# smn-ailab/PyCMF

Hardware: AMD Instinct MI355X
Metric: factor-update iterations/s (mu solver: one full update_step per iteration) (higher is better)
Workload: dtype f32

## Files before the change

pycmf_amd/csrc/cmf_api.hip:

```cpp
#include "../../include/cmfhip.h"
#include "cmf_kernels.hip.h"
#include "cmf_gemm_pair.hip.h"
#include "cmf_eigen.hip.h"
#include "cmf_chol_mfma.hip.h"
#include "cmf_sparse.hip.h"
#include "cmf_rowhess.hip.h"
#include "cmf_bf16x6.hip.h"
#include "cmf_rowhess6.hip.h"
#include "cmf_shared64.hip.h"
#include "cmf_refine64.hip.h"
#include "cmf_eigclamp.hip.h"
#include "cmf_rank1clamp.hip.h"

#include <hip/hip_runtime.h>

#include <algorithm>
#include <chrono>
#include <cmath>
#include <cstdarg>
#include <cstdio>
#include <cstdlib>
#include <cstring>
#include <mutex>
#include <numeric>
#include <set>
#include <string>
#include <thread>
#include <vector>

using namespace cmfk;

static thread_local std::string g_err;

static int fail(int code, const char *fmt, ...) {
    char buf[512];
    va_list ap;
    va_start(ap, fmt);
    vsnprintf(buf, sizeof buf, fmt, ap);
    va_end(ap);
    g_err = buf;
    return code;
}

#define HIPCHK(expr)                                                                       \
    do {                                                                                   \
        hipError_t e_ = (expr);                                                            \
        if (e_ != hipSuccess)                                                              \
            return fail(e_ == hipErrorOutOfMemory ? CMF_ENOMEM : CMF_EHIP, "%s failed: %s (%s:%d)", \
                        #expr, hipGetErrorString(e_), __FILE__, __LINE__);                 \
    } while (0)
#define CHK(expr)                 \
    do {                          \
        int rc_ = (expr);         \
        if (rc_ != CMF_OK) return rc_; \
    } while (0)

static inline int64_t rup(int64_t x, int64_t a) { return (x + a - 1) / a * a; }

struct DevBuf {
    void *p = nullptr;
    size_t bytes = 0;
};

struct CsrDev {
    int64_t *indptr = nullptr;
    int32_t *idx = nullptr;
    float *val = nullptr;
    int64_t rows = 0, cols = 0, nnz = 0;
    cmfk::BcsrEntry *b_ent = nullptr;
    int64_t *b_seg = nullptr;
    int32_t *b_grow = nullptr;
    int b_ngroups = 0, b_nblocks = 0, b_rows_per_group = 0, b_nsync = 1;
    int32_t *b_vmap = nullptr, *b_prow = nullptr, *b_pfirst = nullptr, *b_pcnt = nullptr;
    int b_nsplit = 0, b_nslots = 0;
};

struct WCsrDev {
    int64_t *indptr = nullptr;
    int32_t *idx = nullptr;
    float *pv = nullptr, *wv = nullptr, *tv = nullptr;
    float *ev = nullptr;
    int64_t rows = 0, cols = 0, nnz = 0;
};

struct StepGraph {
    hipGraphExec_t exec = nullptr;
    double key[8] = {0};
    int warm = 0;
    bool failed = false;
};

struct EvPair {
    hipEvent_t a, b;
    int cls;
    double flops;
};

struct CmfComm;
struct cmf_ctx {
    int device = 0;
    CmfComm *comm = nullptr;
    hipStream_t stream = nullptr;
    bool own_stream = false;
    int num_cu = 256;

    int64_t m = 0, d = 0, p = 0;
    int k = 0;
    int64_t mp = 0, dp = 0, pp = 0;
    int kp = 0;
    bool have_problem = false;
    unsigned long long *dbg_stamps = nullptr;
    bool diag_ok = false;
    int opt_graph = -1;
    StepGraph mu_graph, newton_graph;
    int opt_split = -1;
    int opt_pair = 1;
    int opt_arith_min_tiles = 8;
    int opt_arith = 0;
    int opt_ns = 1;
    bool hess_psd = true;
    int opt_pipe_nt = 4;
    int opt_topk_split = 0;
    int opt_kl_split = 0;
    DevBuf kl_slab, kl_small, kl_part;
    int opt_wmu_split = 0;
    int wm_kind[2] = {0, 0};
    float *wm_w[2] = {nullptr, nullptr}, *wm_p[2] = {nullptr, nullptr};
    WCsrDev wm_sp[2][2];
    DevBuf wm_slab, wm_small, wm_part;
    DevBuf hals_ws;
    int opt_als_piece = 0;
    DevBuf als_h, als_part, als_g, als_sol, als_desc;
    DevBuf als_nnls_ws;
    int opt_als_cg_lds = -1;
    DevBuf als_cg_ws;
    int opt_als_cg_piece = 0;
    DevBuf als_cg_long;
    int64_t als_cg_last[2] = {0, 0};
    double wm_bg[2] = {0.0, 0.0};
    DevBuf als_bg_s, als_bg64;
    int opt_choldiag = 0;
    int opt_chol = 1;
    int opt_chol_mfma = 1;
    int opt_zlogit_l2 = 1;
    int opt_rowdiag = 0;
    int opt_rowsym = 4;
    int opt_rowstagger = 1;
    int opt_rowkernel = 1;
    double flop_scale = 1.0;
    bool dev_sampling = false;
    uint64_t dev_seed = 0;
    int64_t sample_off[3] = {0, 0, 0};

    float *X = nullptr, *Y = nullptr;
    CsrDev sp[2][2];
    bool sparse[2] = {false, false};
    double sp_sq[2] = {0.0, 0.0};
    int opt_sparse = 0;
    int opt_spmm_blocked = 1;
    int64_t opt_spmm_block_cols = 0;
    int64_t opt_spmm_stretch = 0;
    DevBuf spmm_bar;
    DevBuf spmm_part;
    int opt_spmm_split = 1;
    float *F[3] = {nullptr, nullptr, nullptr};
    int64_t frows[3] = {0, 0, 0}, frows_pad[3] = {0, 0, 0};
    int64_t v_rows_alloc = 0;

    float *num = nullptr, *den = nullptr;
    float *G = nullptr, *G2 = nullptr, *Hm = nullptr, *Hinv = nullptr, *Eye = nullptr;
    float *vbuf = nullptr;
    DevBuf gslab32;
    int opt_gram32_shares = 32;
    int opt_gram32 = 1;
    DevBuf slabs, slabs_b;
    int slab_sel = 0;
    int timed_open = 0;
    DevBuf narrow_tmp;
    int opt_narrow_update = 1;
    int opt_fused_mu = 1;
    int opt_small_tile = 1;
    DevBuf resid;
    DevBuf resid2, resid3;
    DevBuf kr1, kr2;
    DevBuf hrows;
    DevBuf mask1, mask2;
    DevBuf lists1, lists2;
    DevBuf hpart;
    int opt_rowsplit = 1;
    DevBuf lr_small, lr_rows;
    int opt_lowrank = 1;
    DevBuf lists1s, lists2s, zerobuf;
    DevBuf cls_idx[2], cls_off[2], cls_cnt[2], cls_pat[2], hclass;
    DevBuf certimg, certflag;
    int opt_direct_step = 1;
    int opt_rowcert = 1;
    int64_t opt_rowchunk = 0;
    int opt_rowclasses = -1;
    DevBuf idxbuf;
    DevBuf eigws;
    DevBuf eigflag, eigcopy;
    DevBuf clampstat;
    DevBuf badbuf, rw64, rh64;
    DevBuf ref_w, ref_w2, ref_g, ref_i, ref_ns;
    int opt_refine_batched = 1;
    std::vector<int> bad_host;
    int opt_refine = 1;
    double opt_refine_ratio = 3.0e3;
    double opt_refine_cond = 1.0e3;
    double opt_refine_tol = 2.0e-5;
    int64_t opt_refine_max = (int64_t)1 << 40;
    int64_t refined_sweep = 0, refined_total = 0;
    DevBuf bfp[2][2], bff;
    bool bfp_valid[2][2] = {{false, false}, {false, false}};
    DevBuf nsidx, nsws;
    DevBuf eigcl_snap;
    DevBuf eigcl_ws, eigcl_log, eigcl_fail;
    int opt_eig_clamp = 1;
    int64_t eig_clamp_rows = 0;
    DevBuf r1_ws;
    int opt_rank1_clamp = 1;
    int64_t rank1_rows = 0;
    DevBuf g64a, g64b, gmix64, h64;
    DevBuf gslab64, w64, ns64;
    bool gmix64_valid = false;
    int opt_shared64 = 1;
    DevBuf hinv64, opr;
    int opt_reassoc = 1;
    bool v_plain = false;
    DevBuf dpart;
    int opt_trace_error_off = 0;
    bool mu_dots = false;
    DevBuf trace64;
    double dsq_cache[2] = {0.0, 0.0};
    bool dsq_valid[2] = {false, false};
    double *dscalar = nullptr;
    double rh_credited = 0.0, rh_gathered = 0.0;
    std::vector<void *> owned;
    std::vector<void *> scratch;
    std::set<const void *> lds_opt_in;

    int timing = 0;
    std::vector<EvPair> pending;
    std::vector<hipEvent_t> evpool;
    double ms[CMF_K_END] = {0};
    int64_t launches[CMF_K_END] = {0};
    double flops[CMF_K_END] = {0};
    std::vector<hipEvent_t> markers;
    void *pin[2] = {nullptr, nullptr};
    hipEvent_t pin_ev[2] = {nullptr, nullptr};
    bool pin_busy[2] = {false, false};
    double sp_sum[2] = {0.0, 0.0};
};

struct DeviceGuard {
    int prev = -1;
    explicit DeviceGuard(int dev) {
        (void)hipGetDevice(&prev);
        if (prev != dev) (void)hipSetDevice(dev);
        else prev = -1;
    }
    ~DeviceGuard() {
        if (prev >= 0) (void)hipSetDevice(prev);
    }
};

static int ev_get(cmf_ctx *c, hipEvent_t *e) {
    if (!c->evpool.empty()) {
        *e = c->evpool.back();
        c->evpool.pop_back();
        return CMF_OK;
    }
    HIPCHK(hipEventCreate(e));
    return CMF_OK;
}
struct Timed {
    cmf_ctx *c;
    int cls;
    hipEvent_t a = nullptr, b = nullptr;
    bool on = false;
    double flops = 0.0;
    Timed(cmf_ctx *c_, int cls_, double flops_ = 0.0) : c(c_), cls(cls_), flops(flops_) {
        const bool want = c->timed_open == 0 &&
                          (c->timing == 1 || (c->timing == 2 && (cls == CMF_K_GEMM_NN || cls == CMF_K_GEMM_TN || cls == CMF_K_GEMM_PAIR || cls == CMF_K_SPMM || cls == CMF_K_ROWHESS || cls == CMF_K_KLMU)));
        if (want && ev_get(c, &a) == CMF_OK && ev_get(c, &b) == CMF_OK) {
            on = true;
            ++c->timed_open;
            (void)hipEventRecord(a, c->stream);
        }
    }
    ~Timed() {
        if (on) {
            --c->timed_open;
            (void)hipEventRecord(b, c->stream);
            c->pending.push_back({a, b, cls, flops});
        }
    }
};
static int flush_timing(cmf_ctx *c) {
    if (c->pending.empty()) return CMF_OK;
    HIPCHK(hipStreamSynchronize(c->stream));
    for (auto &e : c->pending) {
        float ms = 0.f;
        HIPCHK(hipEventElapsedTime(&ms, e.a, e.b));
        c->ms[e.cls] += ms;
        c->launches[e.cls] += 1;
        c->flops[e.cls] += e.flops;
        c->evpool.push_back(e.a);
        c->evpool.push_back(e.b);
    }
    c->pending.clear();
    return CMF_OK;
}

static int dev_alloc(cmf_ctx *c, void **p, size_t bytes, bool zero = true) {
    HIPCHK(hipMalloc(p, bytes ? bytes : 16));
    c->owned.push_back(*p);
    if (zero) HIPCHK(hipMemsetAsync(*p, 0, bytes ? bytes : 16, c->stream));
    return CMF_OK;
}
static void dev_free(cmf_ctx *c, void *p) {
    if (!p) return;
    auto it = std::find(c->owned.begin(), c->owned.end(), p);
    if (it != c->owned.end()) c->owned.erase(it);
    (void)hipFree(p);
}
static void drop_graph(StepGraph &g) {
    if (g.exec) (void)hipGraphExecDestroy(g.exec);
    g = StepGraph();
}
static void invalidate_graphs(cmf_ctx *c) {
    drop_graph(c->mu_graph);
    drop_graph(c->newton_graph);
}

static int ensure(cmf_ctx *c, DevBuf &b, size_t bytes) {
    if (b.bytes >= bytes) return CMF_OK;
    invalidate_graphs(c);
    if (b.p) {
        HIPCHK(hipStreamSynchronize(c->stream));
        dev_free(c, b.p);
        b.p = nullptr;
        b.bytes = 0;
    }
    CHK(dev_alloc(c, &b.p, bytes, false));
    b.bytes = bytes;
    return CMF_OK;
}

static int allow_big_lds(cmf_ctx *c, const void *fn, int bytes) {
    if (c->lds_opt_in.count(fn)) return CMF_OK;
    HIPCHK(hipFuncSetAttribute(fn, hipFuncAttributeMaxDynamicSharedMemorySize, bytes));
    c->lds_opt_in.insert(fn);
    return CMF_OK;
}

struct GemmPlan {
    int bn;
    int ntiles_n;
    int64_t tiles_m;
    int nsplit;
    int64_t klen;
};

static GemmPlan plan_gemm(const cmf_ctx *c, int64_t mout, int64_t n, int64_t kred, bool allow_split) {
    GemmPlan pl;
    pl.bn = n >= 256 ? 256 : (int)n;
    pl.ntiles_n = (int)(n / pl.bn);
    pl.tiles_m = (mout + 255) / 256;
    const int64_t tiles = pl.tiles_m * pl.ntiles_n;
    int64_t s = 1;
    if (allow_split && c->opt_split > 0) {
        s = std::min<int64_t>(c->opt_split, std::max<int64_t>(1, kred / 32));
    } else if (allow_split && tiles < (int64_t)(c->num_cu * 3) / 4) {
        s = ((int64_t)c->num_cu + tiles / 2) / tiles;
        const int64_t maxs = std::max<int64_t>(1, kred / 128);
        s = std::max<int64_t>(1, std::min(s, maxs));
    }
    pl.klen = rup((kred + s - 1) / s, 32);
    pl.nsplit = (int)((kred + pl.klen - 1) / pl.klen);
    return pl;
}

template <int MODE, int ROLE>
static int launch_gemm(cmf_ctx *c, const GemmArgs &a, const GemmPlan &pl) {
    static_assert(MODE != MODE_NT, "NT passes: gemm_nt");
    dim3 grid((unsigned)pl.tiles_m, (unsigned)pl.ntiles_n, (unsigned)pl.nsplit);
    dim3 block(512);
#define CMF_LAUNCH(BN_)                                                                          \
    do {                                                                                         \
        using Cfg = GemmCfg<MODE, BN_>;                                                          \
        CHK(allow_big_lds(c, reinterpret_cast<const void *>(&gemm_kernel<MODE, BN_, ROLE, 4>), (int)Cfg::LDS_BYTES)); \
        hipLaunchKernelGGL((gemm_kernel<MODE, BN_, ROLE, 4>), grid, block, Cfg::LDS_BYTES, c->stream, a); \
    } while (0)
    switch (pl.bn) {
    case 256: CMF_LAUNCH(256); break;
    case 128: CMF_LAUNCH(128); break;
    case 64: CMF_LAUNCH(64); break;
    case 32: CMF_LAUNCH(32); break;
    default: return fail(CMF_EINVAL, "unsupported tile width %d", pl.bn);
    }
#undef CMF_LAUNCH
    HIPCHK(hipGetLastError());
    return CMF_OK;
}

static int sum_slabs(cmf_ctx *c, float *dst, const float *src, int64_t n, int nslab, int64_t stride,
                     bool accumulate) {
    Timed tm(c, CMF_K_ELEMWISE);
    const int64_t n4 = n / 4;
    const int blocks = (int)std::min<int64_t>((n4 + 255) / 256, 2048);
    hipLaunchKernelGGL(sum_slabs_kernel, dim3(blocks), dim3(256), 0, c->stream, dst, src, n4, nslab, stride,
                       accumulate ? 1 : 0);
    HIPCHK(hipGetLastError());
    return CMF_OK;
}

static int mu_apply(cmf_ctx *c, float *F, const float *num, const float *den, int64_t n, double l1, double l2);

struct SlabRef {
    const float *base = nullptr;
    int nslab = 0;
    int64_t stride = 0;
    int64_t quota = 0, unit0 = 0;
    int ksteps = 0;
};

struct Epilogue {
    int kind = 0;
    const float *F = nullptr, *P = nullptr;
    const SlabRef *Pslabs = nullptr, *Pslabs2 = nullptr;
    float *out = nullptr;
    double a = 0.0, b = 0.0, c = 0.0;
    int64_t rows = 0;
    int kvalid = 0, nn = 0;
};

static int gemm(cmf_ctx *c, int mode, const float *A, int64_t lda, const float *B, int64_t ldb, float *out,
                int64_t mout, int64_t n, int64_t kred, bool accumulate = false, const Epilogue *mu = nullptr, SlabRef *defer = nullptr) {
    const bool data_pass = (lda != c->kp);
    DevBuf &slabbuf = c->slab_sel ? c->slabs_b : c->slabs;
    if (kred % 32 || n % 32) return fail(CMF_EINVAL, "gemm: unpadded extent (k=%lld n=%lld)", (long long)kred, (long long)n);
    GemmPlan pl = plan_gemm(c, mout, n, kred, mu == nullptr);
    if (mu && c->opt_narrow_update && pl.ntiles_n == 1) {
        while (pl.bn > 64 && pl.tiles_m * (n / pl.bn) * 2 <= (int64_t)c->num_cu) pl.bn /= 2;
        pl.ntiles_n = (int)(n / pl.bn);
    }
    float *alias_out = nullptr;
    if (mu && pl.ntiles_n > 1 && mu->out == A) {
        CHK(ensure(c, c->narrow_tmp, (size_t)rup(mout, 256) * n * sizeof(float)));
        alias_out = mu->out;
    }
    GemmArgs a;
    memset(&a, 0, sizeof a);
    a.A = A; a.lda = lda; a.B = B; a.ldb = ldb;
    a.ldc = n;
    a.Mout = (mode == MODE_TN) ? mout : rup(mout, 256);
    a.Kred = kred; a.klen = pl.klen;
    a.dbg = data_pass ? c->dbg_stamps : nullptr;
    const int64_t rows_store = (mode == MODE_TN) ? mout : rup(mout, 256);
    const bool direct = (pl.nsplit == 1 && !accumulate);
    if (mu) {
        if (mode != MODE_NN || pl.nsplit != 1) return fail(CMF_EINVAL, "fused update needs an unsplit NN product");
        a.epi = mu->kind; a.epi_F = mu->F; a.epi_P = mu->P; a.epi_out = alias_out ? (float *)c->narrow_tmp.p : mu->out;
        a.epi_a = (float)mu->a; a.epi_b = (float)mu->b; a.epi_c = (float)mu->c;
        a.epi_rows = mu->rows; a.epi_kvalid = mu->kvalid; a.epi_nn = mu->nn;
        a.C = out;
    } else if (direct) {
        a.C = out;
        a.slab_stride = 0;
    } else if (pl.nsplit == 1) {
        a.red_out = out; a.red_acc = 1;
        a.C = out;
    } else {
        const size_t need = (size_t)pl.nsplit * rows_store * n * sizeof(float);
        CHK(ensure(c, slabbuf, need));
        a.C = (float *)slabbuf.p;
        a.slab_stride = rows_store * n;
    }
    {
        Timed tm(c, !data_pass ? CMF_K_GEMM_SMALL : (mode == MODE_NN ? CMF_K_GEMM_NN : CMF_K_GEMM_TN),
                 2.0 * (double)mout * (double)n * (double)kred * c->flop_scale);
        if (mode == MODE_NN) {
            if (data_pass) CHK((launch_gemm<MODE_NN, 0>(c, a, pl)));
            else CHK((launch_gemm<MODE_NN, 1>(c, a, pl)));
        } else {
            if (data_pass) CHK((launch_gemm<MODE_TN, 0>(c, a, pl)));
            else CHK((launch_gemm<MODE_TN, 1>(c, a, pl)));
        }
    }
    if (alias_out) HIPCHK(hipMemcpyAsync(alias_out, c->narrow_tmp.p, (size_t)rup(mout, 256) * n * sizeof(float), hipMemcpyDeviceToDevice, c->stream));
    if (!mu && pl.nsplit > 1) {
        if (defer && !accumulate) {
            defer->base = (const float *)slabbuf.p; defer->nslab = pl.nsplit; defer->stride = a.slab_stride;
            return CMF_OK;
        }
        CHK(sum_slabs(c, out, (const float *)slabbuf.p, rows_store * n, pl.nsplit, a.slab_stride, accumulate));
    }
    if (defer) *defer = SlabRef();
    return CMF_OK;
}

static int gram32(cmf_ctx *c, const float *F, int64_t rows_pad, float *G) {
    if (!(c->opt_gram32 && (c->kp == 64 || c->kp == 128) && rows_pad >= 1024))
        return gemm(c, MODE_TN, F, c->kp, F, c->kp, G, c->kp, c->kp, rows_pad);
    const int T = c->kp / 64, ntile = T * (T + 1) / 2;
    int64_t nsplit = std::min<int64_t>(std::max<int64_t>(c->opt_gram32_shares, std::min<int64_t>(256, rows_pad / 1024)), rows_pad / 32);
    const int64_t chunk = rup((rows_pad + nsplit - 1) / nsplit, 32);
    nsplit = (rows_pad + chunk - 1) / chunk;
    CHK(ensure(c, c->gslab32, (size_t)nsplit * ntile * 64 * 64 * sizeof(float)));
    Timed tm(c, CMF_K_GEMM_SMALL, 2.0 * (double)rows_pad * c->kp * c->kp);
    hipLaunchKernelGGL(gram32_partial_kernel, dim3((unsigned)ntile, (unsigned)nsplit), dim3(256), 0, c->stream, F, c->kp, rows_pad, chunk, (float *)c->gslab32.p);
    hipLaunchKernelGGL(gram32_reduce_kernel, dim3((unsigned)std::min(64, (c->kp * c->kp + 255) / 256)), dim3(256), 0, c->stream, (const float *)c->gslab32.p,
                       c->kp, (int)nsplit, G);
    HIPCHK(hipGetLastError());
    return CMF_OK;
}

static bool small_tile_ok(const cmf_ctx *c, int64_t rows_pad) {
    return c->opt_fused_mu && c->opt_small_tile && (c->kp == 64 || c->kp == 128) && rows_pad * c->kp <= ((int64_t)1 << 27);
}
static void factor_update_args(FactorUpdArgs &g, const float *A, const float *B, const Epilogue &e) {
    memset(&g, 0, sizeof g);
    g.A = A; g.B = B; g.epi = e.kind; g.F = e.F; g.P = e.P; g.out = e.out;
    if (e.Pslabs && e.Pslabs->nslab > 0) {
        g.S1 = e.Pslabs->base; g.n1 = e.Pslabs->nslab; g.stride1 = e.Pslabs->stride;
        g.q1 = e.Pslabs->quota; g.u1 = e.Pslabs->unit0; g.ks1 = e.Pslabs->ksteps;
    }
    if (e.Pslabs2 && e.Pslabs2->nslab > 0) {
        g.S2 = e.Pslabs2->base; g.n2 = e.Pslabs2->nslab; g.stride2 = e.Pslabs2->stride;
        g.q2 = e.Pslabs2->quota; g.u2 = e.Pslabs2->unit0; g.ks2 = e.Pslabs2->ksteps;
    }
    g.a = (float)e.a; g.b = (float)e.b; g.c = (float)e.c; g.rows_valid = e.rows; g.kvalid = e.kvalid; g.nn = e.nn;
}
static int factor_update2(cmf_ctx *c, const float *A0, const Epilogue &e0, int64_t rows0, const float *A1, const Epilogue &e1, int64_t rows1, const float *B) {
    FactorUpdArgs g0, g1;
    factor_update_args(g0, A0, B, e0);
    factor_update_args(g1, A1, B, e1);
    Timed tm(c, CMF_K_GEMM_SMALL, 2.0 * (double)(rows0 + rows1) * c->kp * c->kp);
    const size_t lds = (size_t)(128 * 128 + 64 * 132) * sizeof(float);
    CHK(allow_big_lds(c, reinterpret_cast<const void *>(&factor_update2_kernel<128>), (int)lds));
    hipLaunchKernelGGL((factor_update2_kernel<128>), dim3((unsigned)((rows0 + rows1) / 64)), dim3(256), lds, c->stream, g0, g1, (int)(rows0 / 64));
    HIPCHK(hipGetLastError());
    return CMF_OK;
}
static int factor_update(cmf_ctx *c, const float *A, const float *B, const Epilogue &e, int64_t rows_pad) {
    FactorUpdArgs g;
    factor_update_args(g, A, B, e);
    Timed tm(c, CMF_K_GEMM_SMALL, 2.0 * (double)rows_pad * c->kp * c->kp);
    const dim3 grid((unsigned)(rows_pad / 64));
    if (c->kp == 128) {
        const size_t lds = (size_t)(128 * 128 + 64 * 132) * sizeof(float);
        CHK(allow_big_lds(c, reinterpret_cast<const void *>(&factor_update_kernel<128>), (int)lds));
        hipLaunchKernelGGL((factor_update_kernel<128>), grid, dim3(256), lds, c->stream, g);
    } else {
        const size_t lds = (size_t)(64 * 64 + 64 * 68) * sizeof(float);
        hipLaunchKernelGGL((factor_update_kernel<64>), grid, dim3(256), lds, c->stream, g);
    }
    HIPCHK(hipGetLastError());
    return CMF_OK;
}

static int mu_update(cmf_ctx *c, float *F, const float *G, const float *num, int64_t rows_pad, double l1, double l2,
                     const SlabRef *num_slabs = nullptr, const SlabRef *num_slabs2 = nullptr) {
    if (small_tile_ok(c, rows_pad)) {
        Epilogue e;
        e.kind = EPI_MU; e.F = F; e.out = F; e.a = l1; e.b = l2; e.c = 1.1920928955078125e-07;
        e.P = (num_slabs && num_slabs->nslab > 0) ? nullptr : num;
        e.Pslabs = num_slabs; e.Pslabs2 = num_slabs2;
        return factor_update(c, F, G, e, rows_pad);
    }
    if (c->opt_fused_mu && c->kp <= 256) {
        Epilogue e;
        e.kind = EPI_MU; e.F = F; e.P = num; e.out = F; e.a = l1; e.b = l2; e.c = 1.1920928955078125e-07;
        return gemm(c, MODE_NN, F, c->kp, G, c->kp, c->den, rows_pad, c->kp, c->kp, false, &e);
    }
    CHK(gemm(c, MODE_NN, F, c->kp, G, c->kp, c->den, rows_pad, c->kp, c->kp));
    return mu_apply(c, F, num, c->den, rows_pad * c->kp, l1, l2);
}

struct NtOut {
    const float *T = nullptr; int64_t ldt = 0;
    float *R = nullptr; float *W = nullptr; int64_t ldr = 0;
    const uint8_t *mask = nullptr; int64_t ldm = 0;
    double *sq = nullptr;
    float scale_r = 1.f, scale_w = 1.f;
    int link = 0, w_is_slope = 0;
};

static int gemm_nt(cmf_ctx *c, const float *L, int64_t rows_pad, int64_t rows_valid, const float *Rt,
                   int64_t cols_pad, int64_t cols_valid, const NtOut &o) {
    const dim3 grid((unsigned)(rows_pad / 256), (unsigned)(cols_pad / 128), 1);
    GemmArgs a;
    memset(&a, 0, sizeof a);
    a.A = L; a.lda = c->kp; a.B = Rt; a.ldb = c->kp;
    a.Kred = c->kp; a.klen = c->kp; a.Mout = rows_pad;
    a.T = o.T; a.ldt = o.ldt; a.R = o.R; a.W = o.W; a.ldr = o.ldr; a.mask = o.mask; a.ldm = o.ldm;
    a.Mvalid = rows_valid; a.Nvalid = cols_valid;
    a.scale_r = o.scale_r; a.scale_w = o.scale_w; a.link = o.link; a.w_is_slope = o.w_is_slope;
    const int64_t nwg = (int64_t)grid.x * grid.y;
    if (o.sq) {
        CHK(ensure(c, c->dpart, (size_t)nwg * sizeof(double)));
        a.sq_out = (double *)c->dpart.p;
    }
    {
        Timed tm(c, CMF_K_GEMM_NT, 2.0 * (double)rows_valid * (double)cols_valid * (double)c->kp * c->flop_scale);
        using Cfg = GemmCfg<MODE_NT, 128, 2>;
        if (c->opt_pipe_nt == 4) {
            CHK(allow_big_lds(c, reinterpret_cast<const void *>(&gemm_kernel<MODE_NT, 128, 0, 4, 2>), (int)Cfg::LDS_BYTES));
            hipLaunchKernelGGL((gemm_kernel<MODE_NT, 128, 0, 4, 2>), grid, dim3(512), Cfg::LDS_BYTES, c->stream, a);
        } else {
            CHK(allow_big_lds(c, reinterpret_cast<const void *>(&gemm_kernel<MODE_NT, 128, 0, 0, 2>), (int)Cfg::LDS_BYTES));
            hipLaunchKernelGGL((gemm_kernel<MODE_NT, 128, 0, 0, 2>), grid, dim3(512), Cfg::LDS_BYTES, c->stream, a);
        }
        HIPCHK(hipGetLastError());
    }
    if (o.sq) {
        Timed tm(c, CMF_K_ELEMWISE);
        hipLaunchKernelGGL(sum_doubles_kernel, dim3(1), dim3(256), 0, c->stream, (const double *)c->dpart.p, nwg, o.sq);
        HIPCHK(hipGetLastError());
    }
    return CMF_OK;
}

static int mu_apply(cmf_ctx *c, float *F, const float *num, const float *den, int64_t n, double l1, double l2) {
    Timed tm(c, CMF_K_ELEMWISE);
    const int64_t n4 = n / 4;
    const int blocks = (int)std::min<int64_t>((n4 + 255) / 256, 2048);
    hipLaunchKernelGGL(mu_apply_kernel, dim3(blocks), dim3(256), 0, c->stream, F, num, den, n4, (float)l1, (float)l2,
                       1.1920928955078125e-07f);
    HIPCHK(hipGetLastError());
    return CMF_OK;
}

#include "cmf_sparse_host.hip.h"

extern "C" const char *cmf_last_error(void) { return g_err.c_str(); }

#ifndef CMF_SOURCE_HASH
#define CMF_SOURCE_HASH "unstamped"
#endif
static const char g_source_stamp[] = "cmfhip-source-sha256:" CMF_SOURCE_HASH;
extern "C" const char *cmf_source_hash(void) { return g_source_stamp + sizeof("cmfhip-source-sha256:") - 1; }

extern "C" int cmf_device_count(int *count) {
    if (!count) return fail(CMF_EINVAL, "null argument");
    int n = 0;
    if (hipGetDeviceCount(&n) != hipSuccess) n = 0;
    *count = n;
    return CMF_OK;
}

extern "C" int cmf_ctx_create(cmf_ctx **out, int device, void *stream) {
    if (!out) return fail(CMF_EINVAL, "null argument");
    int n = 0;
    if (hipGetDeviceCount(&n) != hipSuccess || n <= 0)
        return fail(CMF_ENODEV, "no HIP device visible: libcmfhip needs an MI355X (gfx950); there is no CPU fallback");
    if (device < 0 || device >= n) return fail(CMF_EINVAL, "device %d out of range (have %d)", device, n);
    DeviceGuard dg(device);
    hipDeviceProp_t prop;
    HIPCHK(hipGetDeviceProperties(&prop, device));
    if (strncmp(prop.gcnArchName, "gfx950", 6) != 0)
        return fail(CMF_ENODEV, "device %d is %s; this library carries gfx950 code only", device, prop.gcnArchName);
    cmf_ctx *c = new cmf_ctx();
    c->device = device;
    c->num_cu = prop.multiProcessorCount > 0 ? prop.multiProcessorCount : 256;
    if (stream) {
        c->stream = (hipStream_t)stream;
    } else {
        hipError_t e = hipStreamCreateWithFlags(&c->stream, hipStreamNonBlocking);
        if (e != hipSuccess) {
            delete c;
            return fail(CMF_EHIP, "hipStreamCreate: %s", hipGetErrorString(e));
        }
        c->own_stream = true;
    }
    c->diag_ok = getenv("CMF_DIAG") != nullptr && atoi(getenv("CMF_DIAG")) != 0;
    void *ds = nullptr;
    int rc = dev_alloc(c, &ds, 8 * sizeof(double));
    if (rc != CMF_OK) {
        delete c;
        return rc;
    }
    c->dscalar = (double *)ds;
    *out = c;
    return CMF_OK;
}

static void release_problem(cmf_ctx *c) {
    (void)hipStreamSynchronize(c->stream);
    invalidate_graphs(c);
    for (void *p : c->owned)
        if (p != (void *)c->dscalar) (void)hipFree(p);
    c->owned.clear();
    c->owned.push_back(c->dscalar);
    c->X = c->Y = nullptr;
    c->F[0] = c->F[1] = c->F[2] = nullptr;
    c->num = c->den = c->G = c->G2 = c->Hm = c->Hinv = c->Eye = c->vbuf = nullptr;
    c->slabs = DevBuf(); c->slabs_b = DevBuf(); c->gslab32 = DevBuf(); c->slab_sel = 0; c->narrow_tmp = DevBuf(); c->resid = DevBuf(); c->resid2 = DevBuf(); c->resid3 = DevBuf(); c->dpart = DevBuf();
    c->kr1 = DevBuf(); c->kr2 = DevBuf(); c->hrows = DevBuf(); c->mask1 = DevBuf(); c->mask2 = DevBuf();
    c->lists1 = DevBuf(); c->lists2 = DevBuf(); c->lists1s = DevBuf(); c->lists2s = DevBuf(); c->zerobuf = DevBuf(); c->lr_small = DevBuf(); c->lr_rows = DevBuf(); c->hpart = DevBuf();
    for (int q = 0; q < 2; ++q) { c->cls_idx[q] = DevBuf(); c->cls_off[q] = DevBuf(); c->cls_cnt[q] = DevBuf(); c->cls_pat[q] = DevBuf(); }
    c->hclass = DevBuf(); c->certimg = DevBuf(); c->certflag = DevBuf();
    c->idxbuf = DevBuf(); c->eigws = DevBuf(); c->eigflag = DevBuf(); c->eigcopy = DevBuf(); c->clampstat = DevBuf(); c->badbuf = DevBuf(); c->rw64 = DevBuf(); c->rh64 = DevBuf(); c->bad_host.clear();
    c->ref_w = DevBuf(); c->ref_w2 = DevBuf(); c->ref_g = DevBuf(); c->ref_i = DevBuf(); c->ref_ns = DevBuf();
    c->trace64 = DevBuf(); c->dsq_valid[0] = c->dsq_valid[1] = false;
    c->nsidx = DevBuf(); c->nsws = DevBuf(); c->eigcl_ws = DevBuf(); c->eigcl_log = DevBuf(); c->eigcl_fail = DevBuf(); c->eigcl_snap = DevBuf(); c->r1_ws = DevBuf();
    c->spmm_bar = DevBuf(); c->spmm_part = DevBuf();
    c->kl_slab = DevBuf(); c->kl_small = DevBuf(); c->kl_part = DevBuf();
    c->wm_slab = DevBuf(); c->wm_small = DevBuf(); c->wm_part = DevBuf();
    c->hals_ws = DevBuf();
    c->als_h = DevBuf(); c->als_part = DevBuf(); c->als_g = DevBuf(); c->als_sol = DevBuf(); c->als_desc = DevBuf(); c->als_nnls_ws = DevBuf(); c->als_cg_ws = DevBuf();
    c->als_cg_long = DevBuf(); c->als_cg_last[0] = c->als_cg_last[1] = 0;
    c->als_bg_s = DevBuf(); c->als_bg64 = DevBuf();
    for (int w = 0; w < 2; ++w) {
        c->wm_bg[w] = 0.0;
        c->wm_kind[w] = 0; c->wm_w[w] = c->wm_p[w] = nullptr;
        c->wm_sp[w][0] = WCsrDev(); c->wm_sp[w][1] = WCsrDev();
    }
    c->g64a = DevBuf(); c->g64b = DevBuf(); c->gmix64 = DevBuf(); c->h64 = DevBuf();
    c->gslab64 = DevBuf(); c->w64 = DevBuf(); c->ns64 = DevBuf();
    c->hinv64 = DevBuf(); c->opr = DevBuf(); c->v_plain = false;
    c->gmix64_valid = false;
    for (int w = 0; w < 2; ++w)
        for (int o = 0; o < 2; ++o) { c->bfp[w][o] = DevBuf(); c->bfp_valid[w][o] = false; }
    c->bff = DevBuf();
    c->have_problem = false;
    for (int w = 0; w < 2; ++w) {
        c->sparse[w] = false;
        c->sp_sq[w] = 0.0;
        for (int t = 0; t < 2; ++t) c->sp[w][t] = CsrDev();
    }
}

static void pin_give(void *p);
extern "C" int cmf_comm_destroy(cmf_ctx *c);
extern "C" int cmf_ctx_destroy(cmf_ctx *c) {
    if (!c) return CMF_OK;
    DeviceGuard dg(c->device);
    (void)cmf_comm_destroy(c);
    release_problem(c);
    for (void *p : c->scratch) (void)hipFree(p);
    c->scratch.clear();
    (void)hipFree(c->dscalar);
    for (auto &e : c->pending) { (void)hipEventDestroy(e.a); (void)hipEventDestroy(e.b); }
    for (auto e : c->evpool) (void)hipEventDestroy(e);
    for (auto e : c->markers) (void)hipEventDestroy(e);
    for (int b = 0; b < 2; ++b) {
        pin_give(c->pin[b]);
        if (c->pin_ev[b]) (void)hipEventDestroy(c->pin_ev[b]);
    }
    if (c->own_stream) (void)hipStreamDestroy(c->stream);
    delete c;
    return CMF_OK;
}

extern "C" int cmf_set_option(cmf_ctx *c, const char *name, int64_t value) {
    if (!c || !name) return fail(CMF_EINVAL, "null argument");
    invalidate_graphs(c);
    if (!strcmp(name, "graph")) {
        c->opt_graph = value < 0 ? -1 : (value != 0);
        return CMF_OK;
    }
    if (!strcmp(name, "gemm_pipe_nt")) {
        c->opt_pipe_nt = (int)value;
    } else if (!strcmp(name, "gemm_split")) {
        c->opt_split = (int)value;
    } else if (!strcmp(name, "small_gram_shares")) {
        c->opt_gram32_shares = (int)std::max<int64_t>(1, std::min<int64_t>(value, 1024));
    } else if (!strcmp(name, "small_gram")) {
        c->opt_gram32 = value != 0;
    } else if (!strcmp(name, "chol_mfma")) {
        c->opt_chol_mfma = value != 0;
    } else if (!strcmp(name, "narrow_update")) {
        c->opt_narrow_update = value != 0;
    } else if (!strcmp(name, "pair_passes")) {
        c->opt_pair = (int)value;
    } else if (!strcmp(name, "z_logit_hessian_l2")) {
        c->opt_zlogit_l2 = value != 0;
    } else if (!strcmp(name, "row_diag")) {
#ifndef CMF_DIAG_BUILD
        if (value != 0) return fail(CMF_EINVAL, "row_diag is a timing-only diagnostic (wrong results) that the default build does not carry: "
                                                "build with `python -m pycmf_amd.build --diag` and set CMF_DIAG=1");
#endif
        if (value != 0 && !c->diag_ok) return fail(CMF_EINVAL, "row_diag is a timing-only diagnostic (wrong results): set CMF_DIAG=1 in the environment to allow it");
        c->opt_rowdiag = (int)value;
    } else if (!strcmp(name, "row_stagger")) {
        c->opt_rowstagger = value != 0;
    } else if (!strcmp(name, "row_symmetric")) {
        c->opt_rowsym = (int)value;
    } else if (!strcmp(name, "row_kernel")) {
        c->opt_rowkernel = value != 0;
    } else if (!strcmp(name, "direct_newton_step")) {
        c->opt_direct_step = value != 0;
    } else if (!strcmp(name, "row_certificates")) {
        c->opt_rowcert = value != 0;
    } else if (!strcmp(name, "row_classes")) {
        if (value < -1 || value > 6) return fail(CMF_EINVAL, "row_classes: -1 (automatic), 0 (off) or 2..6 rows per group");
        c->opt_rowclasses = (int)value;
    } else if (!strcmp(name, "row_chunk")) {
        c->opt_rowchunk = std::max<int64_t>(0, value);
    } else if (!strcmp(name, "sample_row_offset_u")) {
        c->sample_off[CMF_U] = value;
    } else if (!strcmp(name, "sample_row_offset_v")) {
        c->sample_off[CMF_V] = value;
    } else if (!strcmp(name, "sample_row_offset_z")) {
        c->sample_off[CMF_Z] = value;
    } else if (!strcmp(name, "gemm_arith")) {
        if (value != 0 && value != 1) return fail(CMF_EINVAL, "gemm_arith must be 0 (fp32 MFMA) or 1 (bf16x6)");
        c->opt_arith = (int)value;
    } else if (!strcmp(name, "gemm_arith_min_tiles")) {
        c->opt_arith_min_tiles = (int)std::max<int64_t>(1, value);
    } else if (!strcmp(name, "trace_error")) {
        c->opt_trace_error_off = value == 0;
    } else if (!strcmp(name, "eig_clamp")) {
        c->opt_eig_clamp = (int)value;
    } else if (!strcmp(name, "rank1_clamp")) {
        c->opt_rank1_clamp = value != 0;
    } else if (!strcmp(name, "newton_schulz")) {
        c->opt_ns = value != 0;
    } else if (!strcmp(name, "chol_diag")) {
#ifndef CMF_DIAG_BUILD
        if (value != 0) return fail(CMF_EINVAL, "chol_diag is a timing-only diagnostic (wrong results) that the default build does not carry: "
                                                "build with `python -m pycmf_amd.build --diag` and set CMF_DIAG=1");
#endif
        if (value != 0 && !c->diag_ok) return fail(CMF_EINVAL, "chol_diag is a timing-only diagnostic (wrong results): set CMF_DIAG=1 in the environment to allow it");
        c->opt_choldiag = (int)value;
    } else if (!strcmp(name, "safe_inverse_cholesky")) {
        c->opt_chol = value != 0;
    } else if (!strcmp(name, "small_tile_update")) {
        c->opt_small_tile = value != 0;
    } else if (!strcmp(name, "fused_mu_update")) {
        c->opt_fused_mu = value != 0;
    } else if (!strcmp(name, "shared_hessian_f64")) {
        c->opt_shared64 = value != 0;
    } else if (!strcmp(name, "refine_rows")) {
        c->opt_refine = value != 0;
    } else if (!strcmp(name, "refine_rows_batched")) {
        c->opt_refine_batched = value != 0;
    } else if (!strcmp(name, "refine_rows_ratio")) {
        c->opt_refine_ratio = (double)std::max<int64_t>(1, value);
    } else if (!strcmp(name, "refine_rows_cond")) {
        c->opt_refine_cond = (double)std::max<int64_t>(1, value);
    } else if (!strcmp(name, "refine_rows_tol_ppm")) {
        c->opt_refine_tol = 1e-6 * (double)std::max<int64_t>(0, value);
    } else if (!strcmp(name, "refine_rows_max")) {
        c->opt_refine_max = std::max<int64_t>(0, value);
    } else if (!strcmp(name, "row_split")) {
        c->opt_rowsplit = value != 0;
    } else if (!strcmp(name, "lowrank_rows")) {
        if (value < 0 || value > 2) return fail(CMF_EINVAL, "lowrank_rows: 0 off, 1 on (p x p systems through chol_solve_kernel), 2 on (one wave per system in registers: A/B, slower)");
        c->opt_lowrank = (int)value;
    } else if (!strcmp(name, "newton_reassoc")) {
        c->opt_reassoc = value != 0;
    } else if (!strcmp(name, "spmm_blocked")) {
        if (value < 0 || value > 2) return fail(CMF_EINVAL, "spmm_blocked must be 0 (never), 1 (auto) or 2 (always); set before cmf_set_data_csr");
        c->opt_spmm_blocked = (int)value;
    } else if (!strcmp(name, "spmm_split")) {
        c->opt_spmm_split = value != 0;
    } else if (!strcmp(name, "spmm_stretch")) {
        c->opt_spmm_stretch = std::max<int64_t>(0, value);
    } else if (!strcmp(name, "spmm_block_cols")) {
        c->opt_spmm_block_cols = std::max<int64_t>(0, value);
    } else if (!strcmp(name, "kl_split")) {
        c->opt_kl_split = (int)std::max<int64_t>(0, std::min<int64_t>(value, 1 << 20));
    } else if (!strcmp(name, "wmu_split")) {
        c->opt_wmu_split = (int)std::max<int64_t>(0, std::min<int64_t>(value, 1 << 20));
    } else if (!strcmp(name, "als_piece")) {
        c->opt_als_piece = (int)std::max<int64_t>(0, std::min<int64_t>(value, 1 << 20));
    } else if (!strcmp(name, "als_cg_lds")) {
        c->opt_als_cg_lds = (int)std::max<int64_t>(-1, std::min<int64_t>(value, 1 << 20));
    } else if (!strcmp(name, "als_cg_piece")) {
        c->opt_als_cg_piece = (int)std::max<int64_t>(-1, std::min<int64_t>(value, 1 << 30));
    } else if (!strcmp(name, "topk_split")) {
        c->opt_topk_split = (int)std::max<int64_t>(0, std::min<int64_t>(value, 1 << 20));
    } else if (!strcmp(name, "sparse_mode")) {
        if (value < 0 || value > 2) return fail(CMF_EINVAL, "sparse_mode must be 0 (auto), 1 (dense) or 2 (native CSR)");
        c->opt_sparse = (int)value;
    } else {
        return fail(CMF_EINVAL, "unknown option %s", name);
    }
    return CMF_OK;
}

extern "C" int cmf_sync(cmf_ctx *c) {
    if (!c) return fail(CMF_EINVAL, "null context");
    DeviceGuard dg(c->device);
    HIPCHK(hipStreamSynchronize(c->stream));
    return CMF_OK;
}

static int pad_k(int k) {
    if (k <= 32) return 32;
    if (k <= 64) return 64;
    if (k <= 128) return 128;
    return (int)rup(k, 256);
}

extern "C" int cmf_set_problem(cmf_ctx *c, int64_t m, int64_t d, int64_t p, int k) {
    if (!c) return fail(CMF_EINVAL, "null context");
    if (m < 0 || d < 0 || p < 0 || k <= 0) return fail(CMF_EINVAL, "bad problem size m=%lld d=%lld p=%lld k=%d", (long long)m, (long long)d, (long long)p, k);
    DeviceGuard dg(c->device);
    release_problem(c);
    c->m = m; c->d = d; c->p = p; c->k = k;
    c->mp = rup(std::max<int64_t>(m, 1), 256);
    c->dp = rup(std::max<int64_t>(d, 1), 256);
    c->pp = rup(std::max<int64_t>(p, 1), 256);
    c->kp = pad_k(k);
    const int64_t rows[3] = {m, d, p}, rowsp[3] = {c->mp, c->dp, c->pp};
    for (int f = 0; f < 3; ++f) {
        c->frows[f] = rows[f];
        c->frows_pad[f] = rowsp[f];
    }
    CHK(dev_alloc(c, (void **)&c->F[CMF_U], (size_t)(c->mp + c->pp) * c->kp * sizeof(float)));
    c->F[CMF_Z] = c->F[CMF_U] + c->mp * c->kp;
    CHK(dev_alloc(c, (void **)&c->F[CMF_V], (size_t)c->dp * c->kp * sizeof(float)));
    c->v_rows_alloc = c->dp;
    const int64_t rmax = std::max(c->mp, std::max(c->dp, c->pp));
    CHK(dev_alloc(c, (void **)&c->num, (size_t)rmax * c->kp * sizeof(float)));
    CHK(dev_alloc(c, (void **)&c->den, (size_t)rmax * c->kp * sizeof(float)));
    const size_t kk = (size_t)c->kp * c->kp * sizeof(float);
    CHK(dev_alloc(c, (void **)&c->G, kk));
    CHK(dev_alloc(c, (void **)&c->G2, kk));
    CHK(dev_alloc(c, (void **)&c->Hm, kk));
    CHK(dev_alloc(c, (void **)&c->Hinv, kk));
    CHK(dev_alloc(c, (void **)&c->Eye, kk));
    CHK(dev_alloc(c, (void **)&c->vbuf, (size_t)c->dp * c->kp * sizeof(float) + kk));
    c->have_problem = true;
    return CMF_OK;
}

#define NEED_PROBLEM(c)                                                       \
    do {                                                                      \
        if (!(c)) return fail(CMF_EINVAL, "null context");                    \
        if (!(c)->have_problem) return fail(CMF_EINVAL, "cmf_set_problem has not been called"); \
    } while (0)

static int data_dims(cmf_ctx *c, int which, int64_t *rows, int64_t *cols, int64_t *rowsp, int64_t *colsp, float ***slot) {
    if (which == 0) { *rows = c->m; *cols = c->d; *rowsp = c->mp; *colsp = c->dp; *slot = &c->X; }
    else if (which == 1) { *rows = c->d; *cols = c->p; *rowsp = c->dp; *colsp = c->pp; *slot = &c->Y; }
    else return fail(CMF_EINVAL, "which must be 0 (X) or 1 (Y)");
    return CMF_OK;
}

static int ensure_dense(cmf_ctx *c, int which) {
    invalidate_graphs(c);
    c->dsq_valid[which] = false;
    c->bfp_valid[which][0] = c->bfp_valid[which][1] = false;
    int64_t r, cc, rp, cp; float **slot;
    CHK(data_dims(c, which, &r, &cc, &rp, &cp, &slot));
    if (!*slot) CHK(dev_alloc(c, (void **)slot, (size_t)rp * cp * sizeof(float)));
    return CMF_OK;
}

static constexpr size_t PIN_BYTES = (size_t)64 << 20;
static std::mutex g_pin_mu;
static std::vector<void *> g_pin_pool;
static int pin_take(void **p) {
    {
        std::lock_guard<std::mutex> lk(g_pin_mu);
        if (!g_pin_pool.empty()) { *p = g_pin_pool.back(); g_pin_pool.pop_back(); return CMF_OK; }
    }
    HIPCHK(hipHostMalloc(p, PIN_BYTES, hipHostMallocPortable));
    return CMF_OK;
}
static void pin_give(void *p) {
    if (!p) return;
    {
        std::lock_guard<std::mutex> lk(g_pin_mu);
        if (g_pin_pool.size() < 4) { g_pin_pool.push_back(p); return; }
    }
    (void)hipHostFree(p);
}
static int pin_buffers(cmf_ctx *c) {
    for (int b = 0; b < 2; ++b) {
        if (!c->pin[b]) CHK(pin_take(&c->pin[b]));
        if (!c->pin_ev[b]) HIPCHK(hipEventCreateWithFlags(&c->pin_ev[b], hipEventDisableTiming));
    }
    return CMF_OK;
}
template <typename F>
static void parallel_rows(int64_t n, int64_t work_per_row, int want, F &&fn) {
    int nt = (int)std::min<int64_t>(want, std::max<int64_t>(1, (n * work_per_row) >> 19));
    nt = (int)std::min<int64_t>(nt, n);
    if (nt <= 1) { fn((int64_t)0, n); return; }
    std::vector<std::thread> th;
    for (int t = 0; t < nt; ++t) th.emplace_back([&, t]() { fn(n * t / nt, n * (t + 1) / nt); });
    for (auto &x : th) x.join();
}
static int host_threads() {
    const unsigned hc = std::thread::hardware_concurrency();
    return (int)std::min<unsigned>(16, std::max<unsigned>(1, hc));
}

template <typename T>
static int upload_strided(cmf_ctx *c, float *dst, int64_t ld, int64_t rows, int64_t cols, const T *src, int64_t rs, int64_t cs) {
    if (rows == 0 || cols == 0) return CMF_OK;
    CHK(pin_buffers(c));
    const int64_t chunk_rows = std::max<int64_t>(1, std::min<int64_t>(rows, (int64_t)PIN_BYTES / (cols * (int64_t)sizeof(float))));
    if (cols * (int64_t)sizeof(float) > (int64_t)PIN_BYTES) return fail(CMF_EUNSUPPORTED, "row of %lld columns exceeds the staging buffer", (long long)cols);
    const int nthr = host_threads();
    int k = 0;
    for (int64_t r0 = 0; r0 < rows; r0 += chunk_rows, ++k) {
        const int b = k & 1;
        if (c->pin_busy[b]) { HIPCHK(hipEventSynchronize(c->pin_ev[b])); c->pin_busy[b] = false; }
        const int64_t nr = std::min(chunk_rows, rows - r0);
        float *stage = (float *)c->pin[b];
        parallel_rows(nr, cols, nthr, [&](int64_t i0, int64_t i1) {
            for (int64_t i = i0; i < i1; ++i) {
                const T *srow = src + (r0 + i) * rs;
                float *drow = stage + i * cols;
                if (cs == 1) for (int64_t j = 0; j < cols; ++j) drow[j] = (float)srow[j];
                else for (int64_t j = 0; j < cols; ++j) drow[j] = (float)srow[j * cs];
            }
        });
        HIPCHK(hipMemcpy2DAsync(dst + r0 * ld, ld * sizeof(float), stage, cols * sizeof(float), cols * sizeof(float), nr,
                                hipMemcpyHostToDevice, c->stream));
        HIPCHK(hipEventRecord(c->pin_ev[b], c->stream));
        c->pin_busy[b] = true;
    }
    HIPCHK(hipStreamSynchronize(c->stream));
    c->pin_busy[0] = c->pin_busy[1] = false;
    return CMF_OK;
}

template <typename T>
static int download_strided(cmf_ctx *c, const float *srcd, int64_t ld, int64_t rows, int64_t cols, T *dst, int64_t rs, int64_t cs) {
    if (rows == 0 || cols == 0) return CMF_OK;
    CHK(pin_buffers(c));
    if (cols * (int64_t)sizeof(float) > (int64_t)PIN_BYTES) return fail(CMF_EUNSUPPORTED, "row of %lld columns exceeds the staging buffer", (long long)cols);
    const int64_t chunk_rows = std::max<int64_t>(1, std::min<int64_t>(rows, (int64_t)PIN_BYTES / (cols * (int64_t)sizeof(float))));
    const int nthr = host_threads();
    HIPCHK(hipStreamSynchronize(c->stream));
    c->pin_busy[0] = c->pin_busy[1] = false;
    auto issue = [&](int64_t r0, int b) -> int {
        const int64_t nr = std::min(chunk_rows, rows - r0);
        HIPCHK(hipMemcpy2DAsync(c->pin[b], cols * sizeof(float), srcd + r0 * ld, ld * sizeof(float), cols * sizeof(float), nr,
                                hipMemcpyDeviceToHost, c->stream));
        HIPCHK(hipEventRecord(c->pin_ev[b], c->stream));
        return CMF_OK;
    };
    CHK(issue(0, 0));
    int k = 0;
    for (int64_t r0 = 0; r0 < rows; r0 += chunk_rows, ++k) {
        const int b = k & 1;
        if (r0 + chunk_rows < rows) CHK(issue(r0 + chunk_rows, b ^ 1));
        HIPCHK(hipEventSynchronize(c->pin_ev[b]));
        const int64_t nr = std::min(chunk_rows, rows - r0);
        const float *stage = (const float *)c->pin[b];
        parallel_rows(nr, cols, nthr, [&](int64_t i0, int64_t i1) {
            for (int64_t i = i0; i < i1; ++i) {
                T *drow = dst + (r0 + i) * rs;
                const float *srow = stage + i * cols;
                if (cs == 1) for (int64_t j = 0; j < cols; ++j) drow[j] = (T)srow[j];
                else for (int64_t j = 0; j < cols; ++j) drow[j * cs] = (T)srow[j];
            }
        });
    }
    return CMF_OK;
}

template <typename T>
static int set_data(cmf_ctx *c, int which, const T *ptr, int64_t rs, int64_t cs) {
    NEED_PROBLEM(c);
    if (!ptr) return fail(CMF_EINVAL, "null data pointer");
    DeviceGuard dg(c->device);
    int64_t r, cc, rp, cp; float **slot;
    CHK(data_dims(c, which, &r, &cc, &rp, &cp, &slot));
    CHK(ensure_dense(c, which));
    c->sparse[which] = false;
// ... 678 lines not shown
```

Baseline: 15.96.

## Add 256-thread 256x256 MFMA GEMM kernel for NN/TN data passes

Adds a dedicated GEMM kernel with 256-thread workgroups, each wave computing a 128x128 sub-tile through 32x32x2 f32 MFMA. Global loads, LDS stores and MFMA issue are interleaved by hand with sched_barriers, and TN passes read A straight from global into registers. It is used by default for the plain-epilogue data passes whose output rows are a multiple of 256. The aim is more data reuse per thread and better latency hiding than the 512-thread generic kernel, at the cost of higher register pressure (256 accumulator floats per thread) and lower occupancy.

```diff
diff --git a/pycmf_amd/csrc/cmf_api.hip b/pycmf_amd/csrc/cmf_api.hip
--- a/pycmf_amd/csrc/cmf_api.hip
+++ b/pycmf_amd/csrc/cmf_api.hip
@@ -1,5 +1,6 @@
 #include "../../include/cmfhip.h"
 #include "cmf_kernels.hip.h"
+#include "cmf_gemm_wg256.hip.h"
 #include "cmf_gemm_pair.hip.h"
 #include "cmf_eigen.hip.h"
 #include "cmf_chol_mfma.hip.h"
@@ -114,6 +115,7 @@
     int opt_graph = -1;
     StepGraph mu_graph, newton_graph;
     int opt_split = -1;
+    int opt_data_pass_wg = 3;
     int opt_pair = 1;
     int opt_arith_min_tiles = 8;
     int opt_arith = 0;
@@ -386,6 +388,13 @@
 static int launch_gemm(cmf_ctx *c, const GemmArgs &a, const GemmPlan &pl) {
     static_assert(MODE != MODE_NT, "NT passes: gemm_nt");
     dim3 grid((unsigned)pl.tiles_m, (unsigned)pl.ntiles_n, (unsigned)pl.nsplit);
+    if (ROLE == 0 && pl.bn == 256 && (c->opt_data_pass_wg & (MODE == MODE_TN ? 1 : 2)) && a.epi == EPI_NONE && a.Mout % 256 == 0) {
+        using Cfg = Wg256Cfg<MODE>;
+        CHK(allow_big_lds(c, reinterpret_cast<const void *>(&gemm_wg256_kernel<MODE>), (int)Cfg::LDS_BYTES));
+        hipLaunchKernelGGL((gemm_wg256_kernel<MODE>), grid, dim3(Cfg::NT), Cfg::LDS_BYTES, c->stream, a);
+        HIPCHK(hipGetLastError());
+        return CMF_OK;
+    }
     dim3 block(512);
 #define CMF_LAUNCH(BN_)                                                                          \
     do {                                                                                         \
@@ -766,6 +775,9 @@
         c->opt_pipe_nt = (int)value;
     } else if (!strcmp(name, "gemm_split")) {
         c->opt_split = (int)value;
+    } else if (!strcmp(name, "data_pass_wg")) {
+        if (value < 0 || value > 3) return fail(CMF_EINVAL, "data_pass_wg: bit 0 the TN data passes, bit 1 the NN data passes (0..3)");
+        c->opt_data_pass_wg = (int)value;
     } else if (!strcmp(name, "small_gram_shares")) {
         c->opt_gram32_shares = (int)std::max<int64_t>(1, std::min<int64_t>(value, 1024));
     } else if (!strcmp(name, "small_gram")) {
diff --git a/pycmf_amd/csrc/cmf_gemm_wg256.hip.h b/pycmf_amd/csrc/cmf_gemm_wg256.hip.h
--- /dev/null
+++ b/pycmf_amd/csrc/cmf_gemm_wg256.hip.h
@@ -0,0 +1,185 @@
+#pragma once
+#include "cmf_kernels.hip.h"
+
+namespace cmfk {
+
+template <int MODE>
+struct Wg256Cfg {
+    static_assert(MODE == MODE_NN || MODE == MODE_TN, "data passes: NN and TN");
+    static constexpr int BM = 256, BN = 256, BK = 32, PADK = BK + 4, NT = 256;
+    static constexpr int A_ELEMS = (MODE == MODE_NN) ? BM * PADK : 0;
+    static constexpr int B_ELEMS = BK * BN;
+    static constexpr int STAGE = A_ELEMS + B_ELEMS;
+    static constexpr int LD = BK * BN / 4 / NT;
+    static constexpr size_t LDS_BYTES = 2 * STAGE * sizeof(float);
+};
+
+template <int MODE>
+__global__ __launch_bounds__(256) void gemm_wg256_kernel(GemmArgs g) {
+    using C = Wg256Cfg<MODE>;
+    constexpr bool NN = (MODE == MODE_NN);
+    constexpr int NGRP = C::BK / 2;
+    extern __shared__ __attribute__((aligned(16))) float smem[];
+
+    const int t = threadIdx.x;
+    const int lane = t & 63, wid = t >> 6;
+    const int l31 = lane & 31, lh = lane >> 5;
+    const int wrow0 = 128 * (wid >> 1), wcol0 = 128 * (wid & 1);
+
+    const int64_t row0 = (int64_t)blockIdx.x * C::BM;
+    const int64_t n0 = (int64_t)blockIdx.y * C::BN;
+    const int64_t kbeg = (int64_t)blockIdx.z * g.klen;
+    int64_t kend = kbeg + g.klen;
+    if (kend > g.Kred) kend = g.Kred;
+    const int nkt = (int)((kend - kbeg) / C::BK);
+    const int64_t klast = kend - C::BK;
+
+    f32x16 acc[4][4];
+#pragma unroll
+    for (int i = 0; i < 4; ++i)
+#pragma unroll
+        for (int j = 0; j < 4; ++j)
+#pragma unroll
+            for (int r = 0; r < 16; ++r) acc[i][j][r] = 0.0f;
+
+    const int64_t wg_linear = ((int64_t)blockIdx.z * gridDim.y + blockIdx.y) * gridDim.x + blockIdx.x;
+    if (g.dbg && t == 0) {
+        g.dbg[4 * wg_linear + 0] = __builtin_amdgcn_s_memtime();
+        g.dbg[4 * wg_linear + 1] = __builtin_amdgcn_s_memrealtime();
+    }
+
+    f32x4 rb[C::LD], ra[NN ? C::LD : 1];
+    f32x4 xr[NN ? 1 : NGRP];
+    const float *Bg = g.B + (int64_t)wid * g.ldb + n0 + 4 * lane;
+    const float *Ag = NN ? g.A + (row0 + (t >> 3)) * g.lda + 4 * (t & 7) : g.A + (int64_t)lh * g.lda + row0 + wrow0 + 4 * l31;
+    const int b_lds = wid * C::BN + 4 * lane, a_lds = (t >> 3) * C::PADK + 4 * (t & 7);
+
+    auto gload_b = [&](int64_t k0, int p) { rb[p] = *reinterpret_cast<const f32x4 *>(Bg + (k0 + 4 * p) * g.ldb); };
+    auto lstore_b = [&](float *Bs, int p) { *reinterpret_cast<f32x4 *>(Bs + b_lds + 4 * p * C::BN) = rb[p]; };
+    auto gload_a = [&](int64_t k0, int p) { ra[p] = *reinterpret_cast<const f32x4 *>(Ag + 32 * p * g.lda + k0); };
+    auto lstore_a = [&](float *As, int p) { *reinterpret_cast<f32x4 *>(As + a_lds + 32 * p * C::PADK) = ra[p]; };
+    auto gload_x = [&](int64_t k0, int s) { xr[s] = *reinterpret_cast<const f32x4 *>(Ag + (k0 + 2 * s) * g.lda); };
+
+    if (nkt <= 0) return;
+    {
+        float *As0 = smem, *Bs0 = smem + C::A_ELEMS;
+#pragma unroll
+        for (int p = 0; p < C::LD; ++p) {
+            gload_b(kbeg, p);
+            if constexpr (NN) gload_a(kbeg, p);
+        }
+#pragma unroll
+        for (int p = 0; p < C::LD; ++p) {
+            lstore_b(Bs0, p);
+            if constexpr (NN) lstore_a(As0, p);
+        }
+        const int64_t k1 = kbeg + C::BK < klast ? kbeg + C::BK : klast;
+#pragma unroll
+        for (int p = 0; p < C::LD; ++p) {
+            gload_b(k1, p);
+            if constexpr (NN) gload_a(k1, p);
+        }
+        if constexpr (!NN)
+#pragma unroll
+            for (int s = 0; s < NGRP; ++s) gload_x(kbeg, s);
+        __syncthreads();
+        for (int kt = 0; kt < nkt; ++kt) {
+            const float *As = smem + (kt & 1) * C::STAGE, *Bs = As + C::A_ELEMS;
+            float *nAs = smem + ((kt + 1) & 1) * C::STAGE, *nBs = nAs + C::A_ELEMS;
+            int64_t kn1 = kbeg + (int64_t)(kt + 1) * C::BK, kn2 = kn1 + C::BK;
+            kn1 = kn1 < klast ? kn1 : klast;
+            kn2 = kn2 < klast ? kn2 : klast;
+            f32x4 a[NN ? 2 : 1][4], b[2];
+            auto ldb_frag = [&](int sidx) {
+                const int kk = NN ? 8 * (sidx >> 2) + 4 * lh + (sidx & 3) : 2 * sidx + lh;
+                b[sidx & 1] = *reinterpret_cast<const f32x4 *>(Bs + kk * C::BN + wcol0 + 4 * l31);
+            };
+            auto lda_frag = [&](int q) {
+#pragma unroll
+                for (int i = 0; i < 4; ++i)
+                    a[q & 1][i] = *reinterpret_cast<const f32x4 *>(As + (wrow0 + 32 * i + l31) * C::PADK + 4 * (2 * q + lh));
+            };
+            if constexpr (NN) lda_frag(0);
+            ldb_frag(0);
+#pragma unroll
+            for (int sidx = 0; sidx < NGRP; ++sidx) {
+                const int q = sidx >> 2, e = sidx & 3;
+                if (sidx + 1 < NGRP) {
+                    ldb_frag(sidx + 1);
+                    if constexpr (NN)
+                        if (e == 0 && q + 1 < NGRP / 4) lda_frag(q + 1);
+                }
+                __builtin_amdgcn_sched_barrier(0);
+#pragma unroll
+                for (int mi = 0; mi < 16; ++mi) {
+                    const int i = mi >> 2, j = mi & 3;
+                    if constexpr (NN) acc[i][j] = __builtin_amdgcn_mfma_f32_32x32x2f32(a[q & 1][i][e], b[sidx & 1][j], acc[i][j], 0, 0, 0);
+                    else acc[i][j] = __builtin_amdgcn_mfma_f32_32x32x2f32(xr[sidx][i], b[sidx & 1][j], acc[i][j], 0, 0, 0);
+                    if constexpr (NN) {
+                        const int p = mi >> 1;
+                        if (sidx == 0) {
+                            if (mi & 1) lstore_b(nBs, p);
+                            else lstore_a(nAs, p);
+                        } else if (sidx == 1) {
+                            if (mi & 1) gload_b(kn2, p);
+                            else gload_a(kn2, p);
+                        }
+                    } else {
+                        if (sidx == 0 && mi < C::LD) lstore_b(nBs, mi);
+                        if (sidx == 0 && mi >= C::LD) gload_b(kn2, mi - C::LD);
+                    }
+                    __builtin_amdgcn_sched_barrier(0);
+                }
+                if constexpr (!NN) {
+                    gload_x(kn1, sidx);
+                    __builtin_amdgcn_sched_barrier(0);
+                }
+            }
+            __syncthreads();
+        }
+    }
+
+    if (g.dbg && t == 0) {
+        g.dbg[4 * wg_linear + 2] = __builtin_amdgcn_s_memtime();
+        g.dbg[4 * wg_linear + 3] = __builtin_amdgcn_s_memrealtime();
+    }
+    const bool in_red = g.red_out != nullptr;
+    float *Cl = (in_red ? g.red_out : g.C + (int64_t)blockIdx.z * g.slab_stride) +
+                (row0 + wrow0 + (NN ? 4 : 16) * lh) * g.ldc + n0 + wcol0 + 4 * l31;
+    const int ldc = (int)g.ldc;
+    auto rowoff = [&](int i, int r) -> int {
+        const int rr = (r & 3) + 8 * (r >> 2);
+        return (NN ? 32 * i + rr : 4 * rr + i) * ldc;
+    };
+    if (in_red && g.red_acc) {
+#pragma unroll
+        for (int i = 0; i < 4; ++i) {
+#pragma unroll
+            for (int j = 0; j < 4; ++j) asm volatile("" : "+a"(acc[i][j]));
+            f32x4 old[16];
+#pragma unroll
+            for (int r = 0; r < 16; ++r) old[r] = *reinterpret_cast<const f32x4 *>(Cl + rowoff(i, r));
+#pragma unroll
+            for (int r = 0; r < 16; ++r) {
+                f32x4 v = {acc[i][0][r], acc[i][1][r], acc[i][2][r], acc[i][3][r]};
+                v += old[r];
+                *reinterpret_cast<f32x4 *>(Cl + rowoff(i, r)) = v;
+            }
+            __builtin_amdgcn_sched_barrier(0);
+        }
+    } else {
+#pragma unroll
+        for (int i = 0; i < 4; ++i) {
+#pragma unroll
+            for (int j = 0; j < 4; ++j) asm volatile("" : "+a"(acc[i][j]));
+#pragma unroll
+            for (int r = 0; r < 16; ++r) {
+                const f32x4 v = {acc[i][0][r], acc[i][1][r], acc[i][2][r], acc[i][3][r]};
+                *reinterpret_cast<f32x4 *>(Cl + rowoff(i, r)) = v;
+            }
+            __builtin_amdgcn_sched_barrier(0);
+        }
+    }
+}
+
+}
```

New measurement: 16.37 (median of 6 runs). +2.5%, better.
